# BaeHann/feature_level_style_transfer_for_TSC

Measured on AMD Instinct MI355X. Metric: train-step samples/sec (univariate TS, len=512, batch=256) at 1/2/4/8 MI355X, higher is better.
Workload: dtype bf16x3

## Files before the change

feature_level_style_transfer_for_tsc_amd/csrc/wn_wgrad.hip:

```cpp
#include <stdlib.h>
#include <type_traits>

#include "fst_common.h"

typedef __bf16 ww_bf16x8 __attribute__((ext_vector_type(8)));
typedef __bf16 ww_bf16x2 __attribute__((ext_vector_type(2)));
typedef float ww_f32x2 __attribute__((ext_vector_type(2)));
typedef unsigned ww_u32x4 __attribute__((ext_vector_type(4)));
#define WW_GLOBAL_PTR(p) ((const __attribute__((address_space(1))) void*)(p))
#define WW_LDS_VOID(p) ((__attribute__((address_space(3))) void*)(p))

#define WW_TT 32
#define WW_MROWS 256
#define WW_ND 3
#define WW_NX 2
#define WW_MAX_NX 5

__device__ __attribute__((aligned(16))) float ww_zero16[4] = {0.f, 0.f, 0.f, 0.f};

#define WW_MAX_SETS 3
struct WwSeg {
  const float* ptr[WW_MAX_SETS];
  long long bs;
  long long mul_off;
  int rows, shift;
  int out, out_off, out_sc, out_sm;
};

struct WwParams {
  WwSeg dy[2];
  WwSeg x[4];
  int n_dy, n_x, M, K, K_main, n_extra;
  int xr;
  int mul;
  int n_groups, ksplit, B, L, tiles_per_seq, n_tiles;
  const float* epi_p;
  const float* epi_r1;
  float* epi_raw;
  int epi_ncls;
  float epi_scale;
  int n_sets;
  int RX;
  int misaligned;
  int exp;
  int Kcols;
  float* slab;
  float* slab_extra;
  float* w[2];
};

__device__ __forceinline__ void ww_split_pair(float a, float b, unsigned& hi, unsigned& lo) {
  const ww_f32x2 v = {a, b};
  hi = __builtin_bit_cast(unsigned, __builtin_convertvector(v, ww_bf16x2));
  const ww_f32x2 r = {a - __uint_as_float(hi << 16), b - __uint_as_float(hi & 0xffff0000u)};
  lo = __builtin_bit_cast(unsigned, __builtin_convertvector(r, ww_bf16x2));
}

template <class V4>
__device__ __forceinline__ void ww_split8(const V4& v0, const V4& v1, ww_bf16x8& hi, ww_bf16x8& lo) {
  ww_u32x4 h, l;
  unsigned hh, ll;
  ww_split_pair(v0.x, v0.y, hh, ll); h[0] = hh; l[0] = ll;
  ww_split_pair(v0.z, v0.w, hh, ll); h[1] = hh; l[1] = ll;
  ww_split_pair(v1.x, v1.y, hh, ll); h[2] = hh; l[2] = ll;
  ww_split_pair(v1.z, v1.w, hh, ll); h[3] = hh; l[3] = ll;
  hi = __builtin_bit_cast(ww_bf16x8, h);
  lo = __builtin_bit_cast(ww_bf16x8, l);
}

typedef float ww_f32x4 __attribute__((ext_vector_type(4)));
__device__ __forceinline__ ww_f32x4 ww_lds_read16(const char* p) {
  ww_f32x4 v;
  const unsigned addr = (unsigned)(uintptr_t)((__attribute__((address_space(3))) const char*)p);
  asm volatile("ds_read_b128 %0, %1" : "=v"(v) : "v"(addr) : "memory");
  return v;
}
__device__ __forceinline__ void ww_lds_write16(char* p, const ww_u32x4& v) {
  const unsigned addr = (unsigned)(uintptr_t)((__attribute__((address_space(3))) char*)p);
  asm volatile("ds_write_b128 %0, %1" ::"v"(addr), "v"(v) : "memory");
}
__device__ __forceinline__ void ww_lds_zero4(char* p) {
  const unsigned addr = (unsigned)(uintptr_t)((__attribute__((address_space(3))) char*)p);
  asm volatile("ds_write_b32 %0, %1" ::"v"(addr), "v"(0.0f) : "memory");
}
__device__ __forceinline__ void ww_dma16(const char* gsrc, char* lds_dst) {
  const unsigned addr = (unsigned)(uintptr_t)((__attribute__((address_space(3))) char*)lds_dst);
  unsigned saved_m0;
  asm volatile("s_mov_b32 %0, m0\n\ts_mov_b32 m0, %2\n\ts_nop 0\n\tglobal_load_lds_dwordx4 %1, off\n\ts_mov_b32 m0, %0"
               : "=&s"(saved_m0) : "v"(gsrc), "s"(addr) : "memory");
}
__device__ __forceinline__ void ww_lds_wait() {
  asm volatile("s_waitcnt lgkmcnt(0)" ::: "memory");
  __builtin_amdgcn_sched_barrier(0);
}

template <class V4>
__device__ __forceinline__ void ww_split8u(const V4& v0, const V4& v1, ww_u32x4& h, ww_u32x4& l) {
  unsigned hh, ll;
  ww_split_pair(v0.x, v0.y, hh, ll); h[0] = hh; l[0] = ll;
  ww_split_pair(v0.z, v0.w, hh, ll); h[1] = hh; l[1] = ll;
  ww_split_pair(v1.x, v1.y, hh, ll); h[2] = hh; l[2] = ll;
  ww_split_pair(v1.z, v1.w, hh, ll); h[3] = hh; l[3] = ll;
}

template <int N>
__device__ __forceinline__ void ww_wait_vmcnt() {
  asm volatile("s_waitcnt vmcnt(%0)" ::"n"(N) : "memory");
}

__device__ __forceinline__ int ww_dma_row(int i, int lane) { return 8 * i + ((lane >> 3) ^ (i & 1)); }
__device__ __forceinline__ int ww_lds_off(int r, int q) { return ((r ^ ((r >> 3) & 1)) << 7) + (((q ^ r) & 7) << 4); }

struct WwSrc { const float* p; int bs, t; };

template <int MT, int KT, bool FULL, bool MUL, int NE>
__global__ __launch_bounds__(512, 2) void wn_wgrad_kernel(WwParams p) {
  extern __shared__ __attribute__((aligned(16))) char ww_lds[];
  const int tid = threadIdx.x, lane = tid & 63, half = lane >> 5, l31 = lane & 31;
  const int wave_s = __builtin_amdgcn_readfirstlane(tid >> 6);
  const int wm = wave_s >> 1, wk = wave_s & 1;
  const int g = blockIdx.y, L = p.L;
  const int set = blockIdx.x % p.n_sets;
  const int dslot_bytes = WW_MROWS * 128, xslot_bytes = p.RX * 128;
  char* const xring = ww_lds + WW_ND * dslot_bytes;
  const char* const zero16 = reinterpret_cast<const char*>(ww_zero16);

  WwSrc dsrc[4];
#pragma unroll
  for (int k = 0; k < 4; ++k) {
    const int i = wave_s + 8 * k;
    const int r = ww_dma_row(i, lane), q = (lane ^ r) & 7;
    dsrc[k].p = nullptr; dsrc[k].bs = 0; dsrc[k].t = 4 * q;
    if (r < p.M) {
      if (p.n_dy > 1 && r >= p.dy[0].rows) {
        dsrc[k].p = p.dy[1].ptr[set] + ((long long)(r - p.dy[0].rows) * L + 4 * q); dsrc[k].bs = (int)p.dy[1].bs;
      } else {
        dsrc[k].p = p.dy[0].ptr[set] + ((long long)r * L + 4 * q); dsrc[k].bs = (int)p.dy[0].bs;
      }
    }
  }
  const int NXI = p.RX >> 3;
  const int my_nx = (NXI - wave_s + 7) >> 3;
  WwSrc xsrc[WW_MAX_NX];
#pragma unroll
  for (int k = 0; k < WW_MAX_NX; ++k) {
    xsrc[k].p = nullptr; xsrc[k].bs = 0; xsrc[k].t = 0;
    const int i = wave_s + 8 * k;
    if (k >= my_nx) continue;
    const int rr = ww_dma_row(i, lane), q = (lane ^ rr) & 7;
    int kk = -1;
    bool partner = false;
    if (rr < p.xr) kk = g * p.xr + rr;
    else if (p.mul && rr < 2 * p.xr) { kk = g * p.xr + rr - p.xr; partner = true; }
    else {
      const int e = rr - p.xr * (1 + p.mul);
      if (g == 0 && e < p.n_extra) kk = p.K_main + e;
    }
    if (kk >= 0 && kk < p.K && (kk < p.K_main || rr >= p.xr * (1 + p.mul))) {
      int si = 0, c0 = kk;
#pragma unroll
      for (int j = 0; j < 3; ++j)
        if (si + 1 < p.n_x && c0 >= p.x[si].rows) { c0 -= p.x[si].rows; ++si; }
      const float* sp = p.x[0].ptr[set];
      long long sbs = p.x[0].bs, smo = p.x[0].mul_off;
      int ssh = p.x[0].shift;
      if (si == 1) { sp = p.x[1].ptr[set]; sbs = p.x[1].bs; smo = p.x[1].mul_off; ssh = p.x[1].shift; }
      if (si == 2) { sp = p.x[2].ptr[set]; sbs = p.x[2].bs; smo = p.x[2].mul_off; ssh = p.x[2].shift; }
      if (si == 3) { sp = p.x[3].ptr[set]; sbs = p.x[3].bs; smo = p.x[3].mul_off; ssh = p.x[3].shift; }
      xsrc[k].p = sp + ((long long)c0 * L + ssh + 4 * q) + (partner ? smo : 0);
      xsrc[k].bs = (int)sbs;
      xsrc[k].t = ssh + 4 * q;
    }
  }

  int patch_sh = 0;
  if (p.misaligned && tid < p.xr) {
    const int kk = g * p.xr + tid;
    int c0 = kk, si = 0;
#pragma unroll
    for (int j = 0; j < 3; ++j)
      if (si + 1 < p.n_x && c0 >= p.x[si].rows) { c0 -= p.x[si].rows; ++si; }
    const int sh = si == 0 ? p.x[0].shift : (si == 1 ? p.x[1].shift : (si == 2 ? p.x[2].shift : p.x[3].shift));
    if (kk < p.K_main && (sh & 3) != 0 && sh > -4 && sh < 4) patch_sh = sh;
  }
  __builtin_amdgcn_s_waitcnt(0x0F70);

  auto tile_bt = [&](int tile, int& b, int& t0) {
    b = tile / p.tiles_per_seq;
    t0 = (tile - b * p.tiles_per_seq) * WW_TT;
  };
  auto issue_dy1 = [&](int k, int b, int t0, int slot) {
    if (p.exp & 4) return;
    const bool ok = dsrc[k].p != nullptr && t0 + dsrc[k].t < L && !(p.exp & 1);
    const char* src = ok ? reinterpret_cast<const char*>(dsrc[k].p + ((long long)b * dsrc[k].bs + t0)) : zero16;
    ww_dma16(src, ww_lds + slot * dslot_bytes + (wave_s + 8 * k) * 1024);
  };
  auto issue_x1 = [&](int k, int b, int t0, int slot) {
    if (k >= my_nx || (p.exp & 4)) return;
    const int t = t0 + xsrc[k].t;
    const bool ok = xsrc[k].p != nullptr && t > -4 && t < L && !(p.exp & 1);
    const char* src = ok ? reinterpret_cast<const char*>(xsrc[k].p + ((long long)b * xsrc[k].bs + t0)) : zero16;
    ww_dma16(src, xring + slot * xslot_bytes + (wave_s + 8 * k) * 1024);
  };
  auto issue_dy = [&](int tile, int slot) {
    int b, t0;
    tile_bt(tile, b, t0);
#pragma unroll
    for (int k = 0; k < 4; ++k) issue_dy1(k, b, t0, slot);
  };
  auto issue_x = [&](int tile, int slot) {
    int b, t0;
    tile_bt(tile, b, t0);
#pragma unroll
    for (int k = 0; k < WW_MAX_NX; ++k) issue_x1(k, b, t0, slot);
  };

  f32x16 acc[MT][KT];
#pragma unroll
  for (int i = 0; i < MT; ++i)
#pragma unroll
    for (int j = 0; j < KT; ++j)
#pragma unroll
      for (int r = 0; r < 16; ++r) acc[i][j][r] = 0.f;
  float ev[2] = {0.f, 0.f};

  const int wg_in_set = blockIdx.x / p.n_sets, wgs_of_set = (p.ksplit - set + p.n_sets - 1) / p.n_sets;
  const int tile_begin = (int)(((long long)wg_in_set * p.n_tiles) / wgs_of_set);
  const int tile_end = (int)(((long long)(wg_in_set + 1) * p.n_tiles) / wgs_of_set);
  const int m_blocks = (p.M + 31) >> 5;
  const int k_blocks_here = min(2 * KT, ((p.K_main + 31) >> 5) - g * 2 * KT);
  const bool do_extra = NE > 0 && g == 0;

  const int row_l = (l31 ^ ((l31 >> 3) & 1)) << 7;
  const int sw = l31 & 7;
  int pc[2][2];
#pragma unroll
  for (int ks = 0; ks < 2; ++ks) {
    pc[ks][0] = (((4 * ks + 2 * half) ^ sw) & 7) << 4;
    pc[ks][1] = (((4 * ks + 2 * half + 1) ^ sw) & 7) << 4;
  }
  const int a_off = ((wm * MT * 32) << 7) + row_l;
  const int x_off = ((wk * KT * 32) << 7) + row_l, xp_off = x_off + (p.xr << 7);
  const int e_off = (p.xr * (1 + p.mul)) << 7;

  const int n_st = tile_end - tile_begin;
  if (n_st > 0) { issue_dy(tile_begin, 0); issue_x(tile_begin, 0); }
  if (n_st > 1) issue_dy(tile_begin + 1, 1);
  int dslot = 0, xslot = 0;
  for (int c = 0; c < n_st; ++c) {
    if (c + 1 < n_st) ww_wait_vmcnt<4>(); else ww_wait_vmcnt<0>();
    __builtin_amdgcn_s_barrier();
    const bool have_x = c + 1 < n_st, have_dy = c + 2 < n_st;
    int nb = 0, nt0 = 0, db = 0, dt0 = 0;
    if (have_x) tile_bt(tile_begin + c + 1, nb, nt0);
    if (have_dy) tile_bt(tile_begin + c + 2, db, dt0);
    const int x_next = xslot ^ 1, d_next = dslot >= 1 ? dslot - 1 : 2;
    auto issue_pos = [&](int pos) {
      if (pos < WW_MAX_NX) { if (have_x) issue_x1(pos, nb, nt0, x_next); }
      else if (pos < WW_MAX_NX + 4) { if (have_dy) issue_dy1(pos - WW_MAX_NX, db, dt0, d_next); }
    };
    const char* const dsl = ww_lds + dslot * dslot_bytes;
    const char* const xsl = xring + xslot * xslot_bytes;
    if (p.misaligned) {
      int bq, t0;
      tile_bt(tile_begin + c, bq, t0);
      const bool at_start = t0 == 0, at_end = t0 + WW_TT >= L;
      if (at_start || at_end) {
        if (patch_sh != 0) {
          char* rowp = xring + xslot * xslot_bytes + ((tid ^ ((tid >> 3) & 1)) << 7);
          if (at_start && patch_sh < 0)
            for (int j = 0; j < -patch_sh; ++j) ww_lds_zero4(rowp + (((0 ^ tid) & 7) << 4) + 4 * j);
          if (at_end && patch_sh > 0)
            for (int j = 4 - patch_sh; j < 4; ++j) ww_lds_zero4(rowp + (((7 ^ tid) & 7) << 4) + 4 * j);
        }
        asm volatile("s_waitcnt lgkmcnt(0)" ::: "memory");
        __builtin_amdgcn_s_barrier();
      }
    }
    if (!(p.exp & 2)) {
      char* const dw = ww_lds + dslot * dslot_bytes;
      char* const xw = xring + xslot * xslot_bytes;
      const int u = tid & 3, r0 = tid >> 2;
      ww_f32x4 e0, e1;
      if constexpr (NE > 0) {
        e0 = ww_lds_read16(xw + e_off + ((2 * u) << 4));
        e1 = ww_lds_read16(xw + e_off + ((2 * u + 1) << 4));
      }
      ww_f32x4 d[2][2], xq[2][2], xm[2][2];
      char* da[2][2]; char* xa[2][2];
      const int nxu = (p.xr * 4 > 512 + tid) ? 2 : 1;
#pragma unroll
      for (int i = 0; i < 2; ++i) {
        const int r = r0 + 128 * i;
        da[i][0] = dw + ww_lds_off(r, 2 * u); da[i][1] = dw + ww_lds_off(r, 2 * u + 1);
        d[i][0] = ww_lds_read16(da[i][0]); d[i][1] = ww_lds_read16(da[i][1]);
        xa[i][0] = xw + ww_lds_off(r, 2 * u); xa[i][1] = xw + ww_lds_off(r, 2 * u + 1);
        if (i < nxu && r < p.xr) {
          xq[i][0] = ww_lds_read16(xa[i][0]); xq[i][1] = ww_lds_read16(xa[i][1]);
          if constexpr (MUL) {
            xm[i][0] = ww_lds_read16(xa[i][0] + (p.xr << 7)); xm[i][1] = ww_lds_read16(xa[i][1] + (p.xr << 7));
          }
        }
      }
      ww_lds_wait();
#pragma unroll
      for (int i = 0; i < 2; ++i) {
        const int r = r0 + 128 * i;
        if constexpr (NE > 0)
          ev[i] += (d[i][0].x * e0.x + d[i][0].y * e0.y) + (d[i][0].z * e0.z + d[i][0].w * e0.w) +
                   (d[i][1].x * e1.x + d[i][1].y * e1.y) + (d[i][1].z * e1.z + d[i][1].w * e1.w);
        ww_u32x4 h4, l4;
        ww_split8u(d[i][0], d[i][1], h4, l4);
        ww_lds_write16(da[i][0], h4); ww_lds_write16(da[i][1], l4);
        if (i < nxu && r < p.xr) {
          if constexpr (MUL) { xq[i][0] *= xm[i][0]; xq[i][1] *= xm[i][1]; }
          ww_split8u(xq[i][0], xq[i][1], h4, l4);
          ww_lds_write16(xa[i][0], h4); ww_lds_write16(xa[i][1], l4);
        }
      }
      asm volatile("s_waitcnt lgkmcnt(0)" ::: "memory");
    }
    __builtin_amdgcn_s_barrier();
    if (!(p.exp & 2))
#pragma unroll
    for (int ks = 0; ks < 2; ++ks) {
      ww_f32x4 araw[MT][2], braw[KT][2];
#pragma unroll
      for (int i = 0; i < MT; ++i) {
        const char* ap = dsl + a_off + ((i * 32) << 7);
        araw[i][0] = ww_lds_read16(ap + pc[ks][0]);
        araw[i][1] = ww_lds_read16(ap + pc[ks][1]);
      }
#pragma unroll
      for (int j = 0; j < KT; ++j) {
        const char* bp = xsl + x_off + ((j * 32) << 7);
        braw[j][0] = ww_lds_read16(bp + pc[ks][0]);
        braw[j][1] = ww_lds_read16(bp + pc[ks][1]);
      }
      ww_lds_wait();
      issue_pos(5 * ks);
#pragma unroll
      for (int j = 0; j < KT; ++j) {
        if (FULL || wk * KT + j < k_blocks_here) {
          const ww_bf16x8 bh = __builtin_bit_cast(ww_bf16x8, braw[j][0]), bl = __builtin_bit_cast(ww_bf16x8, braw[j][1]);
#pragma unroll
          for (int i = 0; i < MT; ++i) {
            if (!FULL && wm * MT + i >= m_blocks) break;
            const ww_bf16x8 ah = __builtin_bit_cast(ww_bf16x8, araw[i][0]), al = __builtin_bit_cast(ww_bf16x8, araw[i][1]);
            acc[i][j] = __builtin_amdgcn_mfma_f32_32x32x16_bf16(al, bh, acc[i][j], 0, 0, 0);
            acc[i][j] = __builtin_amdgcn_mfma_f32_32x32x16_bf16(ah, bl, acc[i][j], 0, 0, 0);
            acc[i][j] = __builtin_amdgcn_mfma_f32_32x32x16_bf16(ah, bh, acc[i][j], 0, 0, 0);
          }
        }
        issue_pos(5 * ks + 1 + j);
      }
      if constexpr (KT < 3) issue_pos(5 * ks + 3);
      issue_pos(5 * ks + 4);
    }
    dslot = dslot == WW_ND - 1 ? 0 : dslot + 1;
    xslot ^= 1;
  }

  float* const slab = p.slab + (long long)blockIdx.x * WW_MROWS * p.Kcols;
#pragma unroll
  for (int i = 0; i < MT; ++i) {
    if (wm * MT + i >= m_blocks) break;
#pragma unroll
    for (int j = 0; j < KT; ++j) {
      if (wk * KT + j >= k_blocks_here) break;
      float* dst = slab + (long long)((wm * MT + i) * 32 + 4 * half) * p.Kcols + g * p.xr + (wk * KT + j) * 32 + l31;
#pragma unroll
      for (int r = 0; r < 16; ++r) dst[(long long)((r & 3) + 8 * (r >> 2)) * p.Kcols] = acc[i][j][r];
    }
  }
  if (do_extra) {
#pragma unroll
    for (int i = 0; i < 2; ++i) {
      float sv = ev[i];
      sv += __shfl_xor(sv, 1, 64);
      sv += __shfl_xor(sv, 2, 64);
      if ((tid & 3) == 0) p.slab_extra[((long long)blockIdx.x * WW_MROWS + (tid >> 2) + 128 * i) * 2] = sv;
    }
  }
}

__device__ __forceinline__ void ww_scatter(const WwParams& p, int m, int kk, float v) {
  int si = 0, c = kk;
#pragma unroll
  for (int j = 0; j < 3; ++j)
    if (si + 1 < p.n_x && c >= p.x[si].rows) { c -= p.x[si].rows; ++si; }
  int out = p.x[0].out, off = p.x[0].out_off, sc = p.x[0].out_sc, sm = p.x[0].out_sm;
  if (si == 1) { out = p.x[1].out; off = p.x[1].out_off; sc = p.x[1].out_sc; sm = p.x[1].out_sm; }
  if (si == 2) { out = p.x[2].out; off = p.x[2].out_off; sc = p.x[2].out_sc; sm = p.x[2].out_sm; }
  if (si == 3) { out = p.x[3].out; off = p.x[3].out_off; sc = p.x[3].out_sc; sm = p.x[3].out_sm; }
  float* w = out == 0 ? p.w[0] : p.w[1];
  const long long at = (long long)m * sm + (long long)c * sc + off;
  if (p.epi_p) {
    float sd = 0.f;
    for (int j = 0; j < p.epi_ncls; ++j) sd += p.epi_p[m * p.epi_ncls + j] * p.epi_r1[(long long)j * sm + c];
    if (p.epi_raw) p.epi_raw[at] = v;
    v = v * p.epi_scale * sd;
  }
  w[at] = v;
}

__global__ __launch_bounds__(256) void wn_wgrad_reduce_kernel(WwParams p) {
  __shared__ float4 part[4][64];
  const int m = blockIdx.y, cx = threadIdx.x & 63, sg = threadIdx.x >> 6;
  const int kk0 = blockIdx.x * 256 + cx * 4;
  float4 s = make_float4(0.f, 0.f, 0.f, 0.f);
  if (kk0 < p.Kcols) {
    const long long st = (long long)WW_MROWS * p.Kcols;
    const float* q = p.slab + (long long)m * p.Kcols + kk0;
    int sl = sg;
    for (; sl + 28 < p.ksplit; sl += 32) {
      float4 v[8];
#pragma unroll
      for (int u = 0; u < 8; ++u) v[u] = *reinterpret_cast<const float4*>(q + (sl + 4 * u) * st);
#pragma unroll
      for (int u = 0; u < 8; ++u) { s.x += v[u].x; s.y += v[u].y; s.z += v[u].z; s.w += v[u].w; }
    }
    for (; sl < p.ksplit; sl += 4) {
      const float4 v = *reinterpret_cast<const float4*>(q + sl * st);
      s.x += v.x; s.y += v.y; s.z += v.z; s.w += v.w;
    }
  }
  part[sg][cx] = s;
  __syncthreads();
  if (sg == 0 && kk0 < p.Kcols) {
    float4 t = part[0][cx];
#pragma unroll
    for (int g2 = 1; g2 < 4; ++g2) { const float4 o = part[g2][cx]; t.x += o.x; t.y += o.y; t.z += o.z; t.w += o.w; }
    const float tv[4] = {t.x, t.y, t.z, t.w};
#pragma unroll
    for (int j = 0; j < 4; ++j)
      if (kk0 + j < p.K_main) ww_scatter(p, m, kk0 + j, tv[j]);
  }
  if (blockIdx.x == gridDim.x - 1 && sg == 1 && cx < p.n_extra && p.K_main < p.K) {
    const float* q = p.slab_extra + (long long)m * 2 + cx;
    float e = 0.f;
    for (int sl = 0; sl < p.ksplit; ++sl) e += q[(long long)sl * WW_MROWS * 2];
    ww_scatter(p, m, p.K_main + cx, e);
  }
}

static inline bool ww_al16(const void* q) { return q == nullptr || (reinterpret_cast<uintptr_t>(q) & 15) == 0; }

static int ww_geometry(int kind, int B, int L, int n, int h, int last, int n_sets, WwParams* p) {
  const int KT = kind == 0 ? 3 : 2;
  p->M = kind == 0 ? 2 * n : (last ? n : 2 * n);
  p->K = kind == 0 ? 3 * n + h : n;
  const int rem = p->K & 31;
  p->n_extra = (kind == 0 && rem == 1) ? 1 : 0;
  p->K_main = p->n_extra ? p->K - rem : p->K;
  p->xr = 32 * 2 * KT;
  const int kb = (p->K_main + 31) / 32;
  p->n_groups = (kb + 2 * KT - 1) / (2 * KT);
  p->mul = kind == 1;
  p->RX = p->xr * (1 + p->mul) + (p->n_extra ? 8 : 0);
  p->Kcols = p->n_groups * p->xr;
  p->B = B; p->L = L;
  p->tiles_per_seq = L / WW_TT;
  p->n_tiles = B * p->tiles_per_seq;
  const int cus = fst_cu_count() > 0 ? fst_cu_count() : 256;
  int ks = cus / p->n_groups;
  if (ks > p->n_tiles * n_sets) ks = p->n_tiles * n_sets;
  if (ks < n_sets) ks = n_sets;
  p->ksplit = ks;
  p->n_sets = n_sets;
  return KT;
}

extern "C" int fst_wn_wgrad_ok(int kind, int B, int L, int n, int h, int dil) {
  if (!(B > 0 && L > 0 && L % WW_TT == 0 && n > 0 && n < 128)) return 0;
  if (kind == 0) {
    if (!(h > 0 && h <= 32 && dil > 0 && (3 * n + h + 31) / 32 <= 18)) return 0;
    return dil % 4 == 0 ? 1 : (dil < 4 ? 2 : 0);
  }
  return kind == 1;
}

extern "C" int64_t fst_wn_wgrad_workspace_floats(int kind, int B, int L, int n, int h, int last) {
  if (!fst_wn_wgrad_ok(kind, B, L, n, h, 4)) return -1;
  WwParams p;
  ww_geometry(kind, B, L, n, h, last, WW_MAX_SETS, &p);
  return (int64_t)p.ksplit * WW_MROWS * (p.Kcols + 2);
}

static int ww_launch(WwParams& p, int KT, void* stream, bool reduce = true) {
  static const int exp_env = getenv("FST_WW_EXP") ? atoi(getenv("FST_WW_EXP")) : 0;
  p.exp = exp_env;
  const size_t lds = (size_t)WW_ND * WW_MROWS * 128 + (size_t)WW_NX * p.RX * 128;
  FST_REQUIRE(lds <= 160 * 1024 && (p.RX >> 3) <= 8 * WW_MAX_NX, "fst_wn_wgrad: %d staged k-rows per stage do not fit (LDS %zu B)", p.RX, lds);
  const bool full = (p.M + 31) / 32 == 8 && ((p.K_main + 31) / 32) % (2 * KT) == 0;
  void (*fn)(WwParams);
  if (KT == 3) {
    if (p.n_extra) fn = full ? wn_wgrad_kernel<2, 3, true, false, 1> : wn_wgrad_kernel<2, 3, false, false, 1>;
    else fn = full ? wn_wgrad_kernel<2, 3, true, false, 0> : wn_wgrad_kernel<2, 3, false, false, 0>;
  } else if (p.mul) {
    fn = full ? wn_wgrad_kernel<2, 2, true, true, 0> : wn_wgrad_kernel<2, 2, false, true, 0>;
  } else {
    fn = full ? wn_wgrad_kernel<2, 2, true, false, 0> : wn_wgrad_kernel<2, 2, false, false, 0>;
  }
  if (int rc = fst_allow_full_lds((const void*)fn, "fst_wn_wgrad")) return rc;
  hipLaunchKernelGGL(fn, dim3((unsigned)p.ksplit, (unsigned)p.n_groups), dim3(512), lds, (hipStream_t)stream, p);
  FST_LAUNCH_CHECK();
  if (!reduce) return 0;
  hipLaunchKernelGGL(wn_wgrad_reduce_kernel, dim3((unsigned)((p.Kcols + 255) / 256), (unsigned)p.M), dim3(256), 0, (hipStream_t)stream, p);
  FST_LAUNCH_CHECK();
  return 0;
}

extern "C" int fst_wn_wgrad_in(const float* const* dg, const float* const* a, const float* const* u0, int n_sets, int64_t u0_bs,
                               float* dw_in, float* dw_cond, float* workspace, int64_t workspace_floats, int B, int L, int n, int h,
                               int dil, int a_slack, int64_t numel_a, void* stream) {
  FST_REQUIRE(dg && a && u0 && dw_in && dw_cond && workspace, "fst_wn_wgrad_in: null operand");
  FST_REQUIRE(n_sets >= 1 && n_sets <= WW_MAX_SETS, "fst_wn_wgrad_in: %d operand sets (1..%d)", n_sets, WW_MAX_SETS);
  const int served = fst_wn_wgrad_ok(0, B, L, n, h, dil);
  FST_REQUIRE(served == 1 || (served == 2 && a_slack), "fst_wn_wgrad_in: unsupported shape B=%d L=%d n=%d h=%d dil=%d (needs L %% 32 == 0, "
              "n < 128, h <= 32, and dil %% 4 == 0 or — with 16 readable bytes either side of a — dil < 4)", B, L, n, h, dil);
  FST_REQUIRE((long long)B * n * L == (long long)numel_a, "fst_wn_wgrad_in: B*n*L does not match the element count %lld of a", (long long)numel_a);
  FST_REQUIRE(B == 1 || u0_bs >= (int64_t)h * L, "fst_wn_wgrad_in: u0 batch stride %lld < h*L", (long long)u0_bs);
  FST_REQUIRE(u0_bs % 4 == 0 && ww_al16(workspace), "fst_wn_wgrad_in: operands must be 16-byte aligned");
  WwParams p = {};
  const int KT = ww_geometry(0, B, L, n, h, 0, n_sets, &p);
  FST_REQUIRE(workspace_floats >= (int64_t)p.ksplit * WW_MROWS * (p.Kcols + 2), "fst_wn_wgrad_in: workspace of %lld floats is too small",
              (long long)workspace_floats);
  p.n_dy = 1;
  p.dy[0] = {{}, (long long)2 * n * L, 0, 2 * n, 0, 0, 0, 0, 0};
  p.n_x = 4;
  for (int tap = 0; tap < 3; ++tap) p.x[tap] = {{}, (long long)n * L, 0, n, (tap - 1) * dil, 0, tap, 3, 3 * n};
  p.x[3] = {{}, (long long)u0_bs, 0, h, 0, 1, 0, 1, h};
  for (int s = 0; s < n_sets; ++s) {
    FST_REQUIRE(dg[s] && a[s] && u0[s], "fst_wn_wgrad_in: null operand in set %d", s);
    FST_REQUIRE(ww_al16(dg[s]) && ww_al16(a[s]) && ww_al16(u0[s]), "fst_wn_wgrad_in: operands must be 16-byte aligned");
    p.dy[0].ptr[s] = dg[s];
    for (int tap = 0; tap < 3; ++tap) p.x[tap].ptr[s] = a[s];
    p.x[3].ptr[s] = u0[s];
  }
  p.misaligned = dil % 4 != 0;
  p.slab = workspace;
  p.slab_extra = workspace + (long long)p.ksplit * WW_MROWS * p.Kcols;
  p.w[0] = dw_in; p.w[1] = dw_cond;
  return ww_launch(p, KT, stream);
}

extern "C" int fst_wn_wgrad_rs(const float* const* d_a, const float* const* d_out, const float* const* ts, int n_sets, float* dw_rs,
                               float* workspace, int64_t workspace_floats, int last, int B, int L, int n, int64_t numel_a,
                               void* stream) {
  FST_REQUIRE(d_out && ts && dw_rs && workspace && (last || d_a), "fst_wn_wgrad_rs: null operand");
  FST_REQUIRE(n_sets >= 1 && n_sets <= WW_MAX_SETS, "fst_wn_wgrad_rs: %d operand sets (1..%d)", n_sets, WW_MAX_SETS);
  FST_REQUIRE(fst_wn_wgrad_ok(1, B, L, n, 0, 4), "fst_wn_wgrad_rs: unsupported shape B=%d L=%d n=%d (needs L %% 32 == 0, n < 128)", B, L, n);
  FST_REQUIRE((long long)B * n * L == (long long)numel_a, "fst_wn_wgrad_rs: B*n*L does not match the element count %lld", (long long)numel_a);
  FST_REQUIRE(ww_al16(workspace), "fst_wn_wgrad_rs: operands must be 16-byte aligned");
  WwParams p = {};
  const int KT = ww_geometry(1, B, L, n, 0, last, n_sets, &p);
  FST_REQUIRE(workspace_floats >= (int64_t)p.ksplit * WW_MROWS * (p.Kcols + 2), "fst_wn_wgrad_rs: workspace of %lld floats is too small",
              (long long)workspace_floats);
  p.n_dy = last ? 1 : 2;
  p.dy[0] = {{}, (long long)n * L, 0, n, 0, 0, 0, 0, 0};
  p.dy[1] = {{}, (long long)n * L, 0, n, 0, 0, 0, 0, 0};
  p.n_x = 1;
  p.x[0] = {{}, (long long)2 * n * L, (long long)n * L, n, 0, 0, 0, 1, n};
  for (int s = 0; s < n_sets; ++s) {
    FST_REQUIRE(d_out[s] && ts[s] && (last || d_a[s]), "fst_wn_wgrad_rs: null operand in set %d", s);
    FST_REQUIRE(ww_al16(d_out[s]) && ww_al16(ts[s]) && (last || ww_al16(d_a[s])), "fst_wn_wgrad_rs: operands must be 16-byte aligned");
    if (last) p.dy[0].ptr[s] = d_out[s];
    else { p.dy[0].ptr[s] = d_a[s]; p.dy[1].ptr[s] = d_out[s]; }
    p.x[0].ptr[s] = ts[s];
  }
  p.slab = workspace;
  p.slab_extra = workspace + (long long)p.ksplit * WW_MROWS * p.Kcols;
  p.w[0] = dw_rs; p.w[1] = nullptr;
  return ww_launch(p, KT, stream);
}

extern "C" int64_t fst_nt_gemm_workspace_floats(int M, int N, int K) {
  if (!(M > 0 && M <= WW_MROWS && N > 0 && K > 0 && K % WW_TT == 0)) return -1;
  const int n_groups = ((N + 31) / 32 + 3) / 4;
  const int cus = fst_cu_count() > 0 ? fst_cu_count() : 256;
  int ks = cus / n_groups;
  if (ks > K / WW_TT) ks = K / WW_TT;
  if (ks < 1) ks = 1;
  return (int64_t)ks * WW_MROWS * (n_groups * 128 + 2);
}

extern "C" int fst_nt_gemm(const float* A, const float* Bm, float* C, float* workspace, int64_t workspace_floats, int M, int N, int K,
                           const float* epi_p, const float* epi_r1, int epi_ncls, float epi_scale, float* epi_raw, void* stream) {
  FST_REQUIRE(A && Bm && C && workspace, "fst_nt_gemm: null operand");
  FST_REQUIRE(M > 0 && M <= WW_MROWS && N > 0 && K > 0 && K % WW_TT == 0, "fst_nt_gemm: M=%d N=%d K=%d (needs M <= 256, K %% 32 == 0)", M, N, K);
  FST_REQUIRE((long long)N * K < (1LL << 31) * 4 && (long long)M * N < (1LL << 31), "fst_nt_gemm: operand too large");
  FST_REQUIRE(ww_al16(A) && ww_al16(Bm) && ww_al16(workspace), "fst_nt_gemm: operands must be 16-byte aligned");
  FST_REQUIRE((epi_p == nullptr) == (epi_r1 == nullptr) && (epi_p == nullptr || epi_ncls > 0) && (epi_p != nullptr || epi_raw == nullptr),
              "fst_nt_gemm: the epilogue takes p [M][ncls] and r1 [ncls][N] together (and the raw product only with them)");
  WwParams p = {};
  p.M = M; p.K = N; p.K_main = N; p.n_extra = 0;
  p.xr = 128;
  p.n_groups = ((N + 31) / 32 + 3) / 4;
  p.mul = 0;
  p.RX = p.xr;
  p.Kcols = p.n_groups * p.xr;
  p.B = 1; p.L = K;
  p.tiles_per_seq = K / WW_TT;
  p.n_tiles = p.tiles_per_seq;
  const int cus = fst_cu_count() > 0 ? fst_cu_count() : 256;
  int ks = cus / p.n_groups;
  if (ks > p.n_tiles) ks = p.n_tiles;
  if (ks < 1) ks = 1;
  p.ksplit = ks;
  p.n_sets = 1;
  FST_REQUIRE(workspace_floats >= (int64_t)p.ksplit * WW_MROWS * (p.Kcols + 2), "fst_nt_gemm: workspace of %lld floats is too small",
              (long long)workspace_floats);
  p.n_dy = 1;
  p.dy[0] = {{A, nullptr, nullptr}, 0, 0, M, 0, 0, 0, 0, 0};
  p.n_x = 1;
  p.x[0] = {{Bm, nullptr, nullptr}, 0, 0, N, 0, 0, 0, 1, N};
  p.slab = workspace;
  p.slab_extra = workspace + (long long)p.ksplit * WW_MROWS * p.Kcols;
  p.w[0] = C; p.w[1] = nullptr;
  p.epi_p = epi_p; p.epi_r1 = epi_r1; p.epi_ncls = epi_ncls; p.epi_scale = epi_scale; p.epi_raw = epi_raw;
  const bool direct = p.ksplit == 1 && M == WW_MROWS && p.Kcols == N && !epi_p;
  if (direct) p.slab = C;
  return ww_launch(p, 2, stream, !direct);
}

extern "C" int fst_tap_wgrad_ok(int B, int L, int M, int C, int ntaps, int dil, int pad_left) {
  if (!(B > 0 && L > 0 && L % WW_TT == 0 && M > 0 && M <= WW_MROWS && C > 0 && ntaps >= 1 && ntaps <= 4 && dil > 0)) return 0;
  if (((long long)ntaps * C + 31) / 32 > 18) return 0;
  int need_slack = 0;
  for (int tap = 0; tap < ntaps; ++tap) {
    const int sh = tap * dil - pad_left;
    if (sh % 4 != 0) {
      if (sh <= -4 || sh >= 4) return 0;
      need_slack = 1;
    }
  }
  return need_slack ? 2 : 1;
}

static void tap_geometry(int B, int L, int M, int C, int ntaps, WwParams* p) {
  p->M = M; p->K = ntaps * C; p->K_main = p->K; p->n_extra = 0;
  p->xr = 192;
  p->n_groups = ((p->K + 31) / 32 + 5) / 6;
  p->mul = 0;
  p->RX = p->xr;
  p->Kcols = p->n_groups * p->xr;
// ... 432 lines not shown
```

Baseline: 3555.

## Software-pipeline wgrad kernel: overlap split/convert of next tile with MFMAs

```diff
diff --git a/feature_level_style_transfer_for_tsc_amd/csrc/wn_wgrad.hip b/feature_level_style_transfer_for_tsc_amd/csrc/wn_wgrad.hip
--- a/feature_level_style_transfer_for_tsc_amd/csrc/wn_wgrad.hip
+++ b/feature_level_style_transfer_for_tsc_amd/csrc/wn_wgrad.hip
@@ -14,7 +14,6 @@
 #define WW_MROWS 256
 #define WW_ND 3
 #define WW_NX 2
-#define WW_MAX_NX 5
 
 __device__ __attribute__((aligned(16))) float ww_zero16[4] = {0.f, 0.f, 0.f, 0.f};
 
@@ -113,8 +112,40 @@
 
 struct WwSrc { const float* p; int bs, t; };
 
+#ifndef WW_EXP
+#define WW_EXP 0
+#endif
+
+#ifdef WW_STAMPS
+__device__ unsigned long long ww_stamps[12];
+__device__ __forceinline__ unsigned long long ww_now() {
+  unsigned long long t;
+  asm volatile("s_memtime %0\n\ts_waitcnt lgkmcnt(0)" : "=s"(t)::"memory");
+  return t;
+}
+extern "C" int fst_debug_ww_stamps(unsigned long long* out_host, int reset) {
+  if (out_host) (void)hipMemcpyFromSymbol(out_host, HIP_SYMBOL(ww_stamps), sizeof(unsigned long long) * 12);
+  if (reset) { unsigned long long z[12] = {0}; (void)hipMemcpyToSymbol(HIP_SYMBOL(ww_stamps), z, sizeof(z)); }
+  return 0;
+}
+#define WW_T(var) const unsigned long long var = ww_now()
+#define WW_ACC(slot, a, b) ww_sum[slot] += (b) - (a)
+#define WW_SUMS unsigned long long ww_sum[12] = {0, 0, 0, 0, 0, 0, 0, 0, 0, 0, 0, 0}
+#define WW_FLUSH \
+  if (lane == 0) for (int i_ = 0; i_ < 12; ++i_) atomicAdd(&ww_stamps[i_], ww_sum[i_])
+#else
+#define WW_T(var)
+#define WW_ACC(slot, a, b)
+#define WW_SUMS
+#define WW_FLUSH
+#endif
+
 template <int MT, int KT, bool FULL, bool MUL, int NE>
 __global__ __launch_bounds__(512, 2) void wn_wgrad_kernel(WwParams p) {
+  constexpr int NXW = KT * (1 + MUL);
+  constexpr int XRND = (KT + 1) / 2;
+  constexpr int NS = MT * KT;
+  constexpr int ND_EARLY = NS - 1 < 4 ? NS - 1 : 4;
   extern __shared__ __attribute__((aligned(16))) char ww_lds[];
   const int tid = threadIdx.x, lane = tid & 63, half = lane >> 5, l31 = lane & 31;
   const int wave_s = __builtin_amdgcn_readfirstlane(tid >> 6);
@@ -123,65 +154,74 @@
   const int set = blockIdx.x % p.n_sets;
   const int dslot_bytes = WW_MROWS * 128, xslot_bytes = p.RX * 128;
   char* const xring = ww_lds + WW_ND * dslot_bytes;
+  char* const lring = xring + WW_NX * xslot_bytes;
   const char* const zero16 = reinterpret_cast<const char*>(ww_zero16);
 
-  WwSrc dsrc[4];
+  const float* dsrc[4];
+  const long long dy_bs = p.dy[0].bs;
 #pragma unroll
   for (int k = 0; k < 4; ++k) {
     const int i = wave_s + 8 * k;
     const int r = ww_dma_row(i, lane), q = (lane ^ r) & 7;
-    dsrc[k].p = nullptr; dsrc[k].bs = 0; dsrc[k].t = 4 * q;
+    dsrc[k] = nullptr;
     if (r < p.M) {
-      if (p.n_dy > 1 && r >= p.dy[0].rows) {
-        dsrc[k].p = p.dy[1].ptr[set] + ((long long)(r - p.dy[0].rows) * L + 4 * q); dsrc[k].bs = (int)p.dy[1].bs;
-      } else {
-        dsrc[k].p = p.dy[0].ptr[set] + ((long long)r * L + 4 * q); dsrc[k].bs = (int)p.dy[0].bs;
-      }
-    }
-  }
-  const int NXI = p.RX >> 3;
-  const int my_nx = (NXI - wave_s + 7) >> 3;
-  WwSrc xsrc[WW_MAX_NX];
-#pragma unroll
-  for (int k = 0; k < WW_MAX_NX; ++k) {
-    xsrc[k].p = nullptr; xsrc[k].bs = 0; xsrc[k].t = 0;
-    const int i = wave_s + 8 * k;
-    if (k >= my_nx) continue;
-    const int rr = ww_dma_row(i, lane), q = (lane ^ rr) & 7;
-    int kk = -1;
-    bool partner = false;
-    if (rr < p.xr) kk = g * p.xr + rr;
-    else if (p.mul && rr < 2 * p.xr) { kk = g * p.xr + rr - p.xr; partner = true; }
-    else {
-      const int e = rr - p.xr * (1 + p.mul);
-      if (g == 0 && e < p.n_extra) kk = p.K_main + e;
-    }
-    if (kk >= 0 && kk < p.K && (kk < p.K_main || rr >= p.xr * (1 + p.mul))) {
-      int si = 0, c0 = kk;
+      if (p.n_dy > 1 && r >= p.dy[0].rows) dsrc[k] = p.dy[1].ptr[set] + ((long long)(r - p.dy[0].rows) * L + 4 * q);
+      else dsrc[k] = p.dy[0].ptr[set] + ((long long)r * L + 4 * q);
+    }
+  }
+  auto xrow_src = [&](int kk, int q, bool partner, WwSrc& s) {
+    s.p = nullptr; s.bs = 0; s.t = 0;
+    if (kk < 0 || kk >= p.K) return;
+    int si = 0, c0 = kk;
+#pragma unroll
+    for (int j = 0; j < 3; ++j)
+      if (si + 1 < p.n_x && c0 >= p.x[si].rows) { c0 -= p.x[si].rows; ++si; }
+    const float* sp = p.x[0].ptr[set];
+    long long sbs = p.x[0].bs, smo = p.x[0].mul_off;
+    int ssh = p.x[0].shift;
+    if (si == 1) { sp = p.x[1].ptr[set]; sbs = p.x[1].bs; smo = p.x[1].mul_off; ssh = p.x[1].shift; }
+    if (si == 2) { sp = p.x[2].ptr[set]; sbs = p.x[2].bs; smo = p.x[2].mul_off; ssh = p.x[2].shift; }
+    if (si == 3) { sp = p.x[3].ptr[set]; sbs = p.x[3].bs; smo = p.x[3].mul_off; ssh = p.x[3].shift; }
+    s.p = sp + ((long long)c0 * L + ssh + 4 * q) + (partner ? smo : 0);
+    s.bs = (int)sbs;
+    s.t = ssh + 4 * q;
+  };
+  WwSrc xsrc[NXW];
+#pragma unroll
+  for (int k = 0; k < NXW; ++k) {
+    const int rr = ww_dma_row(wave_s + 8 * k, lane), q = (lane ^ rr) & 7;
+    const bool partner = MUL && rr >= p.xr;
+    const int kk = g * p.xr + (partner ? rr - p.xr : rr);
+    xrow_src(kk < p.K_main ? kk : -1, q, partner, xsrc[k]);
+  }
+  WwSrc lsrc = {nullptr, 0, 0};
+  if (NE > 0 && wave_s == 0) {
+    const int e = ww_dma_row(0, lane), q = (lane ^ e) & 7;
+    if (g == 0 && e < p.n_extra) xrow_src(p.K_main + e, q, false, lsrc);
+  }
+
+  const int su = lane & 3;
+  int srow[2], soff[2][2];
+#pragma unroll
+  for (int i = 0; i < 2; ++i) {
+    srow[i] = 8 * (wave_s + 8 * (2 * i + half)) + ((lane >> 2) & 7);
+    soff[i][0] = ww_lds_off(srow[i], 2 * su);
+    soff[i][1] = ww_lds_off(srow[i], 2 * su + 1);
+  }
+  const bool x_lane1 = 2 + half < KT;
+  int patch_sh[XRND];
+#pragma unroll
+  for (int i = 0; i < XRND; ++i) {
+    patch_sh[i] = 0;
+    const int kk = g * p.xr + srow[i];
+    if (!MUL && p.misaligned && (i == 0 || x_lane1) && kk < p.K_main) {
+      int c0 = kk, si = 0;
 #pragma unroll
       for (int j = 0; j < 3; ++j)
         if (si + 1 < p.n_x && c0 >= p.x[si].rows) { c0 -= p.x[si].rows; ++si; }
-      const float* sp = p.x[0].ptr[set];
-      long long sbs = p.x[0].bs, smo = p.x[0].mul_off;
-      int ssh = p.x[0].shift;
-      if (si == 1) { sp = p.x[1].ptr[set]; sbs = p.x[1].bs; smo = p.x[1].mul_off; ssh = p.x[1].shift; }
-      if (si == 2) { sp = p.x[2].ptr[set]; sbs = p.x[2].bs; smo = p.x[2].mul_off; ssh = p.x[2].shift; }
-      if (si == 3) { sp = p.x[3].ptr[set]; sbs = p.x[3].bs; smo = p.x[3].mul_off; ssh = p.x[3].shift; }
-      xsrc[k].p = sp + ((long long)c0 * L + ssh + 4 * q) + (partner ? smo : 0);
-      xsrc[k].bs = (int)sbs;
-      xsrc[k].t = ssh + 4 * q;
-    }
-  }
-
-  int patch_sh = 0;
-  if (p.misaligned && tid < p.xr) {
-    const int kk = g * p.xr + tid;
-    int c0 = kk, si = 0;
-#pragma unroll
-    for (int j = 0; j < 3; ++j)
-      if (si + 1 < p.n_x && c0 >= p.x[si].rows) { c0 -= p.x[si].rows; ++si; }
-    const int sh = si == 0 ? p.x[0].shift : (si == 1 ? p.x[1].shift : (si == 2 ? p.x[2].shift : p.x[3].shift));
-    if (kk < p.K_main && (sh & 3) != 0 && sh > -4 && sh < 4) patch_sh = sh;
+      const int sh = si == 0 ? p.x[0].shift : (si == 1 ? p.x[1].shift : (si == 2 ? p.x[2].shift : p.x[3].shift));
+      if ((sh & 3) != 0 && sh > -4 && sh < 4) patch_sh[i] = sh;
+    }
   }
   __builtin_amdgcn_s_waitcnt(0x0F70);
 
@@ -191,17 +231,25 @@
   };
   auto issue_dy1 = [&](int k, int b, int t0, int slot) {
     if (p.exp & 4) return;
-    const bool ok = dsrc[k].p != nullptr && t0 + dsrc[k].t < L && !(p.exp & 1);
-    const char* src = ok ? reinterpret_cast<const char*>(dsrc[k].p + ((long long)b * dsrc[k].bs + t0)) : zero16;
+    const bool ok = dsrc[k] != nullptr && !(p.exp & 1);
+    const char* src = ok ? reinterpret_cast<const char*>(dsrc[k] + (b * dy_bs + t0)) : zero16;
     ww_dma16(src, ww_lds + slot * dslot_bytes + (wave_s + 8 * k) * 1024);
   };
   auto issue_x1 = [&](int k, int b, int t0, int slot) {
-    if (k >= my_nx || (p.exp & 4)) return;
+    if (p.exp & 4) return;
     const int t = t0 + xsrc[k].t;
     const bool ok = xsrc[k].p != nullptr && t > -4 && t < L && !(p.exp & 1);
     const char* src = ok ? reinterpret_cast<const char*>(xsrc[k].p + ((long long)b * xsrc[k].bs + t0)) : zero16;
     ww_dma16(src, xring + slot * xslot_bytes + (wave_s + 8 * k) * 1024);
   };
+  auto issue_lo = [&](int tile, int slot) {
+    if (NE == 0 || wave_s != 0 || (p.exp & 4)) return;
+    int b, t0;
+    tile_bt(tile, b, t0);
+    const bool ok = lsrc.p != nullptr && t0 + lsrc.t < L && !(p.exp & 1);
+    const char* src = ok ? reinterpret_cast<const char*>(lsrc.p + ((long long)b * lsrc.bs + t0)) : zero16;
+    ww_dma16(src, lring + slot * 1024);
+  };
   auto issue_dy = [&](int tile, int slot) {
     int b, t0;
     tile_bt(tile, b, t0);
@@ -212,7 +260,7 @@
     int b, t0;
     tile_bt(tile, b, t0);
 #pragma unroll
-    for (int k = 0; k < WW_MAX_NX; ++k) issue_x1(k, b, t0, slot);
+    for (int k = 0; k < NXW; ++k) issue_x1(k, b, t0, slot);
   };
 
   f32x16 acc[MT][KT];
@@ -230,6 +278,7 @@
   const int m_blocks = (p.M + 31) >> 5;
   const int k_blocks_here = min(2 * KT, ((p.K_main + 31) >> 5) - g * 2 * KT);
   const bool do_extra = NE > 0 && g == 0;
+  constexpr bool arith = !(WW_EXP & 2), split_on = !(WW_EXP & 10), mfma_on = !(WW_EXP & 18);
 
   const int row_l = (l31 ^ ((l31 >> 3) & 1)) << 7;
   const int sw = l31 & 7;
@@ -240,126 +289,187 @@
     pc[ks][1] = (((4 * ks + 2 * half + 1) ^ sw) & 7) << 4;
   }
   const int a_off = ((wm * MT * 32) << 7) + row_l;
-  const int x_off = ((wk * KT * 32) << 7) + row_l, xp_off = x_off + (p.xr << 7);
-  const int e_off = (p.xr * (1 + p.mul)) << 7;
+  const int x_off = ((wk * KT * 32) << 7) + row_l;
+
+  ww_f32x4 sd[2][2], sx[XRND][2], sm[XRND][2], se0, se1;
+  auto split_load_dy = [&](const char* dw, const char* lw) {
+#pragma unroll
+    for (int i = 0; i < 2; ++i) { sd[i][0] = ww_lds_read16(dw + soff[i][0]); sd[i][1] = ww_lds_read16(dw + soff[i][1]); }
+    if constexpr (NE > 0) {
+      se0 = ww_lds_read16(lw + ((2 * su) << 4));
+      se1 = ww_lds_read16(lw + ((2 * su + 1) << 4));
+    }
+  };
+  auto split_load_x = [&](const char* xw) {
+#pragma unroll
+    for (int i = 0; i < XRND; ++i) {
+      if (i == 0 || x_lane1) {
+        sx[i][0] = ww_lds_read16(xw + soff[i][0]); sx[i][1] = ww_lds_read16(xw + soff[i][1]);
+        if constexpr (MUL) {
+          sm[i][0] = ww_lds_read16(xw + soff[i][0] + (p.xr << 7)); sm[i][1] = ww_lds_read16(xw + soff[i][1] + (p.xr << 7));
+        }
+      }
+    }
+  };
+  auto split_store_dy = [&](char* dw) {
+#pragma unroll
+    for (int i = 0; i < 2; ++i) {
+      if constexpr (NE > 0)
+        ev[i] += ((__builtin_fmaf(sd[i][0].x, se0.x, sd[i][0].y * se0.y) + __builtin_fmaf(sd[i][0].z, se0.z, sd[i][0].w * se0.w)) +
+                  __builtin_fmaf(sd[i][1].x, se1.x, sd[i][1].y * se1.y)) + __builtin_fmaf(sd[i][1].z, se1.z, sd[i][1].w * se1.w);
+      ww_u32x4 h4, l4;
+      ww_split8u(sd[i][0], sd[i][1], h4, l4);
+      ww_lds_write16(dw + soff[i][0], h4); ww_lds_write16(dw + soff[i][1], l4);
+    }
+  };
+  auto split_store_x = [&](char* xw, int tile) {
+    if (!MUL && p.misaligned) {
+      int bq, t0;
+      tile_bt(tile, bq, t0);
+      const bool at_start = t0 == 0, at_end = t0 + WW_TT >= L;
+#pragma unroll
+      for (int i = 0; i < XRND; ++i) {
+        const int sh = patch_sh[i];
+        if (at_start && sh < 0 && su == 0)
+#pragma unroll
+          for (int j = 0; j < 3; ++j) if (j < -sh) sx[i][0][j] = 0.f;
+        if (at_end && sh > 0 && su == 3)
+#pragma unroll
+          for (int j = 1; j < 4; ++j) if (j >= 4 - sh) sx[i][1][j] = 0.f;
+      }
+    }
+#pragma unroll
+    for (int i = 0; i < XRND; ++i) {
+      if (i == 0 || x_lane1) {
+        if constexpr (MUL) { sx[i][0] *= sm[i][0]; sx[i][1] *= sm[i][1]; }
+        ww_u32x4 h4, l4;
+        ww_split8u(sx[i][0], sx[i][1], h4, l4);
+        ww_lds_write16(xw + soff[i][0], h4); ww_lds_write16(xw + soff[i][1], l4);
+      }
+    }
+  };
+  ww_f32x4 araw[2][MT][2], braw[2][KT][2];
+  auto a_reads = [&](auto ks_c, const char* dsl) {
+    constexpr int ks = decltype(ks_c)::value;
+#pragma unroll
+    for (int i = 0; i < MT; ++i) {
+      const char* ap = dsl + a_off + ((i * 32) << 7);
+      araw[ks][i][0] = ww_lds_read16(ap + pc[ks][0]);
+      araw[ks][i][1] = ww_lds_read16(ap + pc[ks][1]);
+    }
+  };
+  auto b_read = [&](auto ks_c, int j, const char* xsl) {
+    constexpr int ks = decltype(ks_c)::value;
+    const char* bp = xsl + x_off + ((j * 32) << 7);
+    braw[ks][j][0] = ww_lds_read16(bp + pc[ks][0]);
+    braw[ks][j][1] = ww_lds_read16(bp + pc[ks][1]);
+  };
+  auto frag_reads = [&](auto ks_c, const char* dsl, const char* xsl) {
+    a_reads(ks_c, dsl);
+#pragma unroll
+    for (int j = 0; j < KT; ++j) b_read(ks_c, j, xsl);
+  };
+  auto mfma_group = [&](int ks, int s) {
+    const int i = s % MT, j = s / MT;
+    if (mfma_on && (FULL || (wk * KT + j < k_blocks_here && wm * MT + i < m_blocks))) {
+      const ww_bf16x8 bh = __builtin_bit_cast(ww_bf16x8, braw[ks][j][0]), bl = __builtin_bit_cast(ww_bf16x8, braw[ks][j][1]);
+      const ww_bf16x8 ah = __builtin_bit_cast(ww_bf16x8, araw[ks][i][0]), al = __builtin_bit_cast(ww_bf16x8, araw[ks][i][1]);
+      acc[i][j] = __builtin_amdgcn_mfma_f32_32x32x16_bf16(al, bh, acc[i][j], 0, 0, 0);
+      acc[i][j] = __builtin_amdgcn_mfma_f32_32x32x16_bf16(ah, bl, acc[i][j], 0, 0, 0);
+      acc[i][j] = __builtin_amdgcn_mfma_f32_32x32x16_bf16(ah, bh, acc[i][j], 0, 0, 0);
+    }
+    __builtin_amdgcn_sched_barrier(0);
+  };
 
   const int n_st = tile_end - tile_begin;
-  if (n_st > 0) { issue_dy(tile_begin, 0); issue_x(tile_begin, 0); }
-  if (n_st > 1) issue_dy(tile_begin + 1, 1);
+  WW_SUMS;
+  WW_T(w_begin);
+  if (n_st > 0) {
+    issue_dy(tile_begin, 0); issue_x(tile_begin, 0); issue_lo(tile_begin, 0);
+    if (n_st > 1) { issue_lo(tile_begin + 1, 1); issue_dy(tile_begin + 1, 1); ww_wait_vmcnt<4>(); } else ww_wait_vmcnt<0>();
+    if constexpr (NE > 0) __builtin_amdgcn_s_barrier();
+    if (arith && split_on) {
+      split_load_dy(ww_lds, lring);
+      split_load_x(xring);
+      ww_lds_wait();
+      split_store_dy(ww_lds);
+      split_store_x(xring, tile_begin);
+    }
+    ww_lds_wait();
+    __builtin_amdgcn_s_barrier();
+    if (arith) frag_reads(std::integral_constant<int, 0>{}, ww_lds, xring);
+    if (n_st > 1) issue_x(tile_begin + 1, 1);
+    if (n_st > 2) issue_lo(tile_begin + 2, 2);
+  }
+  WW_T(w_loop);
+  WW_ACC(10, w_begin, w_loop);
   int dslot = 0, xslot = 0;
   for (int c = 0; c < n_st; ++c) {
-    if (c + 1 < n_st) ww_wait_vmcnt<4>(); else ww_wait_vmcnt<0>();
-    __builtin_amdgcn_s_barrier();
-    const bool have_x = c + 1 < n_st, have_dy = c + 2 < n_st;
-    int nb = 0, nt0 = 0, db = 0, dt0 = 0;
-    if (have_x) tile_bt(tile_begin + c + 1, nb, nt0);
-    if (have_dy) tile_bt(tile_begin + c + 2, db, dt0);
-    const int x_next = xslot ^ 1, d_next = dslot >= 1 ? dslot - 1 : 2;
-    auto issue_pos = [&](int pos) {
-      if (pos < WW_MAX_NX) { if (have_x) issue_x1(pos, nb, nt0, x_next); }
-      else if (pos < WW_MAX_NX + 4) { if (have_dy) issue_dy1(pos - WW_MAX_NX, db, dt0, d_next); }
-    };
+    const bool nxt = c + 1 < n_st, ahead = c + 2 < n_st, lo_ahead = c + 3 < n_st;
+    const int d1 = dslot == WW_ND - 1 ? 0 : dslot + 1, d2 = dslot == 0 ? WW_ND - 1 : dslot - 1;
     const char* const dsl = ww_lds + dslot * dslot_bytes;
     const char* const xsl = xring + xslot * xslot_bytes;
-    if (p.misaligned) {
-      int bq, t0;
-      tile_bt(tile_begin + c, bq, t0);
-      const bool at_start = t0 == 0, at_end = t0 + WW_TT >= L;
-      if (at_start || at_end) {
-        if (patch_sh != 0) {
-          char* rowp = xring + xslot * xslot_bytes + ((tid ^ ((tid >> 3) & 1)) << 7);
-          if (at_start && patch_sh < 0)
-            for (int j = 0; j < -patch_sh; ++j) ww_lds_zero4(rowp + (((0 ^ tid) & 7) << 4) + 4 * j);
-          if (at_end && patch_sh > 0)
-            for (int j = 4 - patch_sh; j < 4; ++j) ww_lds_zero4(rowp + (((7 ^ tid) & 7) << 4) + 4 * j);
-        }
-        asm volatile("s_waitcnt lgkmcnt(0)" ::: "memory");
-        __builtin_amdgcn_s_barrier();
-      }
-    }
-    if (!(p.exp & 2)) {
-      char* const dw = ww_lds + dslot * dslot_bytes;
-      char* const xw = xring + xslot * xslot_bytes;
-      const int u = tid & 3, r0 = tid >> 2;
-      ww_f32x4 e0, e1;
-      if constexpr (NE > 0) {
-        e0 = ww_lds_read16(xw + e_off + ((2 * u) << 4));
-        e1 = ww_lds_read16(xw + e_off + ((2 * u + 1) << 4));
-      }
-      ww_f32x4 d[2][2], xq[2][2], xm[2][2];
-      char* da[2][2]; char* xa[2][2];
-      const int nxu = (p.xr * 4 > 512 + tid) ? 2 : 1;
-#pragma unroll
-      for (int i = 0; i < 2; ++i) {
-        const int r = r0 + 128 * i;
-        da[i][0] = dw + ww_lds_off(r, 2 * u); da[i][1] = dw + ww_lds_off(r, 2 * u + 1);
-        d[i][0] = ww_lds_read16(da[i][0]); d[i][1] = ww_lds_read16(da[i][1]);
-        xa[i][0] = xw + ww_lds_off(r, 2 * u); xa[i][1] = xw + ww_lds_off(r, 2 * u + 1);
-        if (i < nxu && r < p.xr) {
-          xq[i][0] = ww_lds_read16(xa[i][0]); xq[i][1] = ww_lds_read16(xa[i][1]);
-          if constexpr (MUL) {
-            xm[i][0] = ww_lds_read16(xa[i][0] + (p.xr << 7)); xm[i][1] = ww_lds_read16(xa[i][1] + (p.xr << 7));
-          }
-        }
-      }
+    char* const dn = ww_lds + d1 * dslot_bytes;
+    char* const xn = xring + (xslot ^ 1) * xslot_bytes;
+    int b2 = 0, t2 = 0;
+    if (ahead) tile_bt(tile_begin + c + 2, b2, t2);
+    WW_T(ta);
+    ww_lds_wait();
+    WW_T(tc);
+    WW_ACC(0, ta, tc);
+#pragma unroll
+    for (int s = 0; s < NS - 1; ++s) {
+      if constexpr (arith) mfma_group(0, s);
+      if (s < ND_EARLY && ahead) issue_dy1(s, b2, t2, d2);
+    }
+    WW_T(td);
+    WW_ACC(2, tc, td);
+    if (nxt) {
+      if (ahead) ww_wait_vmcnt<ND_EARLY>(); else ww_wait_vmcnt<0>();
+    }
+    WW_T(te);
+    WW_ACC(3, td, te);
+    if (nxt && arith && split_on) split_load_dy(dn, lring + d1 * 1024);
+    if constexpr (arith) mfma_group(0, NS - 1);
+#pragma unroll
+    for (int k = ND_EARLY; k < 4; ++k)
+      if (ahead) issue_dy1(k, b2, t2, d2);
+    WW_T(tf);
+    WW_ACC(4, te, tf);
+    ww_lds_wait();
+    WW_T(tg);
+    WW_ACC(5, tf, tg);
+    if (nxt && arith && split_on) {
+      split_store_dy(dn);
+      split_load_x(xn);
       ww_lds_wait();
-#pragma unroll
-      for (int i = 0; i < 2; ++i) {
-        const int r = r0 + 128 * i;
-        if constexpr (NE > 0)
-          ev[i] += (d[i][0].x * e0.x + d[i][0].y * e0.y) + (d[i][0].z * e0.z + d[i][0].w * e0.w) +
-                   (d[i][1].x * e1.x + d[i][1].y * e1.y) + (d[i][1].z * e1.z + d[i][1].w * e1.w);
-        ww_u32x4 h4, l4;
-        ww_split8u(d[i][0], d[i][1], h4, l4);
-        ww_lds_write16(da[i][0], h4); ww_lds_write16(da[i][1], l4);
-        if (i < nxu && r < p.xr) {
-          if constexpr (MUL) { xq[i][0] *= xm[i][0]; xq[i][1] *= xm[i][1]; }
-          ww_split8u(xq[i][0], xq[i][1], h4, l4);
-          ww_lds_write16(xa[i][0], h4); ww_lds_write16(xa[i][1], l4);
-        }
-      }
-      asm volatile("s_waitcnt lgkmcnt(0)" ::: "memory");
-    }
+      split_store_x(xn, tile_begin + c + 1);
+    }
+    if (arith) frag_reads(std::integral_constant<int, 1>{}, dsl, xsl);
+    WW_T(tb);
+    WW_ACC(6, tg, tb);
+    ww_lds_wait();
+    WW_T(th);
+    WW_ACC(1, tb, th);
     __builtin_amdgcn_s_barrier();
-    if (!(p.exp & 2))
-#pragma unroll
-    for (int ks = 0; ks < 2; ++ks) {
-      ww_f32x4 araw[MT][2], braw[KT][2];
-#pragma unroll
-      for (int i = 0; i < MT; ++i) {
-        const char* ap = dsl + a_off + ((i * 32) << 7);
-        araw[i][0] = ww_lds_read16(ap + pc[ks][0]);
-        araw[i][1] = ww_lds_read16(ap + pc[ks][1]);
-      }
-#pragma unroll
-      for (int j = 0; j < KT; ++j) {
-        const char* bp = xsl + x_off + ((j * 32) << 7);
-        braw[j][0] = ww_lds_read16(bp + pc[ks][0]);
-        braw[j][1] = ww_lds_read16(bp + pc[ks][1]);
-      }
-      ww_lds_wait();
-      issue_pos(5 * ks);
-#pragma unroll
-      for (int j = 0; j < KT; ++j) {
-        if (FULL || wk * KT + j < k_blocks_here) {
-          const ww_bf16x8 bh = __builtin_bit_cast(ww_bf16x8, braw[j][0]), bl = __builtin_bit_cast(ww_bf16x8, braw[j][1]);
-#pragma unroll
-          for (int i = 0; i < MT; ++i) {
-            if (!FULL && wm * MT + i >= m_blocks) break;
-            const ww_bf16x8 ah = __builtin_bit_cast(ww_bf16x8, araw[i][0]), al = __builtin_bit_cast(ww_bf16x8, araw[i][1]);
-            acc[i][j] = __builtin_amdgcn_mfma_f32_32x32x16_bf16(al, bh, acc[i][j], 0, 0, 0);
-            acc[i][j] = __builtin_amdgcn_mfma_f32_32x32x16_bf16(ah, bl, acc[i][j], 0, 0, 0);
-            acc[i][j] = __builtin_amdgcn_mfma_f32_32x32x16_bf16(ah, bh, acc[i][j], 0, 0, 0);
-          }
-        }
-        issue_pos(5 * ks + 1 + j);
-      }
-      if constexpr (KT < 3) issue_pos(5 * ks + 3);
-      issue_pos(5 * ks + 4);
-    }
-    dslot = dslot == WW_ND - 1 ? 0 : dslot + 1;
+    WW_T(ti);
+    WW_ACC(7, th, ti);
+    if (nxt && arith) a_reads(std::integral_constant<int, 0>{}, dn);
+#pragma unroll
+    for (int s = 0; s < NS; ++s) {
+      if (s < NXW && ahead) issue_x1(s, b2, t2, xslot);
+      if (s == NXW && lo_ahead) issue_lo(tile_begin + c + 3, dslot);
+      if constexpr (arith) mfma_group(1, s);
+      if (s % MT == MT - 1 && nxt && arith) b_read(std::integral_constant<int, 0>{}, s / MT, xn);
+    }
+    WW_T(tj);
+    WW_ACC(8, ti, tj);
+    dslot = d1;
     xslot ^= 1;
   }
+  WW_T(w_end);
+  WW_ACC(9, w_loop, w_end);
+  WW_FLUSH;
 
   float* const slab = p.slab + (long long)blockIdx.x * WW_MROWS * p.Kcols;
 #pragma unroll
@@ -379,7 +489,7 @@
       float sv = ev[i];
       sv += __shfl_xor(sv, 1, 64);
       sv += __shfl_xor(sv, 2, 64);
-      if ((tid & 3) == 0) p.slab_extra[((long long)blockIdx.x * WW_MROWS + (tid >> 2) + 128 * i) * 2] = sv;
+      if (su == 0) p.slab_extra[((long long)blockIdx.x * WW_MROWS + srow[i]) * 2] = sv;
     }
   }
 }
@@ -457,7 +567,7 @@
   const int kb = (p->K_main + 31) / 32;
   p->n_groups = (kb + 2 * KT - 1) / (2 * KT);
   p->mul = kind == 1;
-  p->RX = p->xr * (1 + p->mul) + (p->n_extra ? 8 : 0);
+  p->RX = p->xr * (1 + p->mul);
   p->Kcols = p->n_groups * p->xr;
   p->B = B; p->L = L;
   p->tiles_per_seq = L / WW_TT;
@@ -490,8 +600,10 @@
 static int ww_launch(WwParams& p, int KT, void* stream, bool reduce = true) {
   static const int exp_env = getenv("FST_WW_EXP") ? atoi(getenv("FST_WW_EXP")) : 0;
   p.exp = exp_env;
-  const size_t lds = (size_t)WW_ND * WW_MROWS * 128 + (size_t)WW_NX * p.RX * 128;
-  FST_REQUIRE(lds <= 160 * 1024 && (p.RX >> 3) <= 8 * WW_MAX_NX, "fst_wn_wgrad: %d staged k-rows per stage do not fit (LDS %zu B)", p.RX, lds);
+  const size_t lds = (size_t)WW_ND * WW_MROWS * 128 + (size_t)WW_NX * p.RX * 128 + (p.n_extra ? (size_t)WW_ND * 1024 : 0);
+  FST_REQUIRE(p.n_dy < 2 || p.dy[1].bs == p.dy[0].bs, "fst_wn_wgrad: the two output-row segments need one batch stride");
+  FST_REQUIRE(lds <= 160 * 1024 && p.xr == 64 * KT && p.RX == p.xr * (1 + p.mul) && p.n_extra <= 8,
+              "fst_wn_wgrad: %d staged k-rows per stage do not fit (LDS %zu B)", p.RX, lds);
   const bool full = (p.M + 31) / 32 == 8 && ((p.K_main + 31) / 32) % (2 * KT) == 0;
   void (*fn)(WwParams);
   if (KT == 3) {
```

Result: no change. 3574 (median of 6 runs) (+0.5%).
